# divortio/divortio-lz4

Measured on NVIDIA B200. Metric: lz4_block_roundtrip_throughput, higher is better.
Workload: dtype u8

## Files before the change

divortio-lz4_b200/csrc/api_launch.inc:

```
int compress_segmented(dlz4_ctx *ctx, const uint8_t *d_work, int64_t start, int64_t total, int64_t B, uint32_t n, bool linked,
                       const int32_t *init_table, uint8_t *d_comp, const uint64_t *d_coff, uint32_t *d_clen, cudaStream_t st,
                       int32_t *final_table = nullptr, const uint32_t *landed = nullptr, int32_t land_origin = 0,
                       uint32_t land_shift = 0);

int launch_compress(dlz4_ctx *ctx, const uint8_t *src, const uint64_t *src_off, const uint32_t *src_len, uint32_t n,
                    uint32_t max_len, const uint8_t *prefix, uint32_t prefix_len, const int32_t *init_table, uint8_t *dst,
                    const uint64_t *dst_off, uint32_t *comp_len, cudaStream_t st, uint32_t *counter = nullptr, bool dense = false) {
    if (n == 0) return DLZ4_OK;
    if (!counter) counter = ctx->d_counter;
    CK(cudaMemsetAsync(counter, 0, sizeof(uint32_t), st));
    if (init_table == nullptr) { prefix = nullptr; prefix_len = 0; }
    if (max_len <= 65536 && prefix_len == 0 && init_table == nullptr && ctx->split && n <= kMaxSplitBlocks) {
        const size_t region = (size_t)(counter - ctx->d_counter) % kGtabRegions;
        const uint64_t rstride = (uint64_t)max_len / 4 + 2;
        const size_t region_bytes = (((size_t)n * rstride * 8) * 9 / 8 + 255) & ~(size_t)255;
        if (ctx->rec.cap < region_bytes * kGtabRegions + 256) {
            CK(cudaDeviceSynchronize());
            CKS(reserve(ctx, ctx->rec, std::max(region_bytes, (size_t)ctx->rec.cap / kGtabRegions) * kGtabRegions));
        }
        const size_t per_region = ((ctx->rec.cap - 256) / kGtabRegions) & ~(size_t)255;
        uint64_t *recs = (uint64_t *)((uint8_t *)ctx->rec.p + region * per_region);
        uint32_t *nrec = ctx->d_nrec + region * (size_t)kMaxSplitBlocks;
        if (ctx->probe) CK(cudaEventRecord(ctx->evq[0], st));
        if (ctx->pw) {
            const int grid = (int)std::min<uint64_t>(n, (uint64_t)ctx->sm_count);
            const uint32_t lead = (uint32_t)ctx->pw_lead, ns = (uint32_t)ctx->pw_sleep;
            k_parse_pw<<<grid, kPwThreads, kPwSmemBytes, st>>>(src, src_off, src_len, n, recs, rstride, nrec, counter, lead, ns);
        } else
        {
            const int grid = (int)std::min<uint64_t>((n + kWarpsFresh16 - 1) / kWarpsFresh16, (uint64_t)ctx->sm_count);
            k_parse_fresh16<kWarpsFresh16><<<grid, kWarpsFresh16 * 32, kWarpsFresh16 * kHashEntries * 2, st>>>(
                src, src_off, src_len, n, recs, rstride, nrec, counter);
        }
        if (ctx->probe) CK(cudaEventRecord(ctx->evq[1], st));
        CK(cudaMemsetAsync(counter, 0, sizeof(uint32_t), st));
        const int egrid = (int)std::min<uint64_t>((n + kWarpsDecode - 1) / kWarpsDecode, (uint64_t)ctx->sm_count * 8);
        k_encode_blocks<kWarpsDecode><<<egrid, kWarpsDecode * 32, 0, st>>>(src, src_off, src_len, n, recs, rstride, nrec, dst, dst_off,
                                                                            comp_len, counter);
        if (ctx->probe) CK(cudaEventRecord(ctx->evq[2], st));
        ctx->launches++;
    } else if (max_len <= 65536 && prefix_len == 0 && init_table == nullptr && ctx->hybrid) {
        const size_t region = (size_t)(counter - ctx->d_counter) % kGtabRegions;
        const int grid = (int)std::min<uint64_t>(dense ? (n + kHyWarps - 1) / kHyWarps : n, (uint64_t)ctx->hy_grid);
        uint32_t active = dense ? (uint32_t)kHyWarps : (uint32_t)std::min<uint64_t>((n + grid - 1) / grid, (uint64_t)kHyWarps);
        if (ctx->hy_active) active = std::min<uint32_t>(active, (uint32_t)ctx->hy_active);
        k_compress_fresh16h<<<grid, kHyWarps * 32, kHySmemBytes, st>>>(
            src, src_off, src_len, n, dst, dst_off, comp_len, counter,
            ctx->d_gtabs + region * (size_t)ctx->hy_grid * kHyGlWarps * kHashEntries, active);
    } else if (max_len <= 4096 && prefix_len > 0 && init_table != nullptr && ctx->hybrid && prefix_len < 0x7FFF0000u) {
        const size_t region = (size_t)(counter - ctx->d_counter) % kGtabRegions;
        const int grid = (int)std::min<uint64_t>(dense ? (n + kHyWarps - 1) / kHyWarps : n, (uint64_t)ctx->hy_grid);
        const uint32_t active = dense ? (uint32_t)kHyWarps : (uint32_t)std::min<uint64_t>((n + grid - 1) / grid, (uint64_t)kHyWarps);
        k_compress_overlay<<<grid, kHyWarps * 32, kHySmemBytes, st>>>(
            src, src_off, src_len, n, prefix, prefix_len, init_table, dst, dst_off, comp_len, counter,
            ctx->d_gtabs + region * (size_t)ctx->hy_grid * kHyGlWarps * kHashEntries, active);
    } else {
        if (max_len > 65536 && prefix_len == 0 && init_table == nullptr && n <= 65536) {
            std::vector<uint64_t> off(n);
            std::vector<uint32_t> len(n);
            CK(cudaMemcpyAsync(off.data(), src_off, (size_t)n * 8, cudaMemcpyDeviceToHost, st));
            CK(cudaMemcpyAsync(len.data(), src_len, (size_t)n * 4, cudaMemcpyDeviceToHost, st));
            CK(cudaStreamSynchronize(st));
            const uint64_t B = len[0];
            bool uniform = B > 65536 && (B & (B - 1)) == 0 && off[0] + (uint64_t)n * B < 0x7FFFFFF0ull;
            for (uint32_t i = 0; uniform && i < n; ++i)
                uniform = off[i] == off[0] + (uint64_t)i * B && (len[i] == B || (i + 1 == n && len[i] <= B && len[i] > 0));
            if (uniform) {
                const int64_t total = (int64_t)(n - 1) * (int64_t)B + len[n - 1];
                return compress_segmented(ctx, src, (int64_t)off[0], total, (int64_t)B, n, false, nullptr, dst, dst_off, comp_len, st);
            }
        }
        const int grid = (int)std::min<uint64_t>((n + kWarpsGeneric32 - 1) / kWarpsGeneric32, (uint64_t)ctx->sm_count);
        k_compress_generic32<kWarpsGeneric32><<<grid, kWarpsGeneric32 * 32, kWarpsGeneric32 * (kHashEntries * 4 + kRingBytes), st>>>(
            src, src_off, src_len, n, prefix, prefix_len, init_table, dst, dst_off, comp_len, counter);
    }
    ctx->launches++;
    CK(cudaGetLastError());
    return DLZ4_OK;
}

int launch_decompress(dlz4_ctx *ctx, const uint8_t *src, const uint64_t *src_off, const uint32_t *src_len, uint32_t n,
                      uint8_t *dst, const uint64_t *dst_off, const uint32_t *dst_cap, const uint8_t *dict, uint32_t dict_len,
                      int hist_frame, const uint8_t *stored, uint32_t *out_len, uint8_t *status, cudaStream_t st,
                      uint32_t *counter = nullptr) {
    if (n == 0) return DLZ4_OK;
    if (!counter) counter = ctx->d_counter;
    CK(cudaMemsetAsync(counter, 0, sizeof(uint32_t), st));
    const int grid = hist_frame ? 1 : (int)std::min<uint64_t>((n + kWarpsDecode - 1) / kWarpsDecode, (uint64_t)ctx->sm_count * 8);
    if (dict_len)
        k_decompress_blocks<kWarpsDecode, true><<<grid, hist_frame ? 32 : kWarpsDecode * 32, 0, st>>>(src, src_off, src_len, n, dst, dst_off, dst_cap,
                                                                                                      dict, dict_len, hist_frame, stored, out_len, status, counter);
    else
        k_decompress_blocks<kWarpsDecode, false><<<grid, hist_frame ? 32 : kWarpsDecode * 32, 0, st>>>(src, src_off, src_len, n, dst, dst_off, dst_cap,
                                                                                                       dict, dict_len, hist_frame, stored, out_len, status, counter);
    ctx->launches++;
    CK(cudaGetLastError());
    return DLZ4_OK;
}

int launch_xxh32_batch(dlz4_ctx *ctx, const uint8_t *base, const uint64_t *off, const uint32_t *len, uint32_t n, uint32_t seed,
                       uint32_t *out, uint8_t *append_base, cudaStream_t st) {
    if (n == 0) return DLZ4_OK;
    const uint64_t threads = (uint64_t)n * 4;
    k_xxh32_batch<<<(unsigned)((threads + 255) / 256), 256, 0, st>>>(base, off, len, n, seed, out, append_base);
    ctx->launches++;
    CK(cudaGetLastError());
    return DLZ4_OK;
}

int launch_xxh32_stream(dlz4_ctx *ctx, const uint8_t *data, uint64_t len, uint32_t seed, uint32_t *out, cudaStream_t st) {
    k_xxh32_stream<1><<<1, 32, 0, st>>>(data, len, seed, out, nullptr, nullptr);
    ctx->launches++;
    CK(cudaGetLastError());
    return DLZ4_OK;
}
```

divortio-lz4_b200/csrc/dlz4_parse.cuh:

```cuda
#pragma once

namespace dlz4 {

__device__ __forceinline__ uint2 rec_pack(uint32_t pos, uint32_t ml, uint32_t offset) { return make_uint2(pos | (offset << 16), ml); }

template <class Tab>
__device__ uint32_t parse_block64_warp(const uint8_t *__restrict__ base, const int32_t start, const int32_t len, Tab &T,
                                       uint64_t *__restrict__ rec) {
    const uint32_t lane = lane_id();
    const uint32_t lt = (1u << lane) - 1u;
    const int32_t sEnd = start + len;
    const int32_t mflimit = sEnd - 12;
    const int32_t matchLimit = sEnd - 5;
    int32_t sIndex = start;
    uint32_t smc = 67;
    uint32_t nrec = 0;
    const SrcFlat S{base};

    const uint32_t A0 = (uint32_t)(reinterpret_cast<uintptr_t>(base) & 127u);
    const int32_t wlo = start - (int32_t)((A0 + (uint32_t)start) & 3u);
    const int32_t whi = sEnd;
    uint32_t R0 = 0, R1 = 0, R2 = 0, R3 = 0;
    uint32_t Lc = 0;
    bool cold = true;
// ... 88 lines not shown
            uint32_t mlxa = mla, mlxb = mlb;
            uint32_t cur = 0;
            while (hl < 64u) {
                const uint32_t pk = __shfl_sync(FULL, pack, hl);
                const uint32_t fld = (pk >> ((hl >> 1) & 16u)) & 0xFFFFu;
                uint32_t mlh = fld & 63u;
                uint32_t nxt = fld >> 6;
                if (mlh == 32u && matchLimit - (w + (int32_t)hl) > 32) {
                    const int32_t s0 = w + (int32_t)hl;
                    const int32_t m0 = __shfl_sync(FULL, (hl & 32u) ? candb : canda, hl);
                    for (int32_t eb = 32;; eb += 128) {
                        const int32_t q = s0 + eb + 4 * (int32_t)lane;
                        int32_t nv = matchLimit - q;
                        nv = nv > 4 ? 4 : nv;
                        int32_t eq = 0;
                        if (nv > 0) {
                            const uint32_t x = S.ld32(q) ^ S.ld32(m0 + eb + 4 * (int32_t)lane);
                            eq = x ? ((__ffs(x) - 1) >> 3) : 4;
                            eq = eq < nv ? eq : nv;
                        }
                        const uint32_t stop = __ballot_sync(FULL, eq < 4);
                        if (stop) {
                            const int l = __ffs(stop) - 1;
                            mlh = (uint32_t)(eb + 4 * l + __shfl_sync(FULL, eq, l));
                            break;
                        }
                    }
                    nxt = first_hit_from(hl + mlh);
                    if (lane == (hl & 31u)) { if (hl & 32u) mlxb = mlh; else mlxa = mlh; }
                }
                if (lane == (hl & 31u)) myhead |= 1u + (hl >> 5);
                cur = hl + mlh;
                hl = nxt;
            }
            const uint32_t stop = any_head ? trunc : min(trunc, dl0);
            const uint32_t Ha = __ballot_sync(FULL, myhead & 1u), Hb = __ballot_sync(FULL, myhead & 2u);
            const uint32_t enda = min(lane + mlxa, 255u), endb = min(lane + 32u + mlxb, 255u);
            const uint32_t ends = enda | (endb << 8);
            const uint32_t ma_lo = Ha & lt, mb_lo = Hb & lt;
            const int pha = ma_lo ? 31 - __clz(ma_lo) : -1;
            const int phb = mb_lo ? 63 - __clz(mb_lo) : (Ha ? 31 - __clz(Ha) : -1);
            const uint32_t ea = __shfl_sync(FULL, ends, pha & 31), eb2 = __shfl_sync(FULL, ends, phb & 31);
            const uint32_t end_pha = pha < 0 ? 0u : (ea & 255u);
            const uint32_t end_phb = phb < 0 ? 0u : (phb >= 32 ? eb2 >> 8 : eb2 & 255u);
            const bool ina = lane < end_pha, inb = lane + 32u < end_phb;
            const bool pra = lane < stop && !ina;
            const bool prb = lane + 32u < stop && !inb;
            if (conf) {
                if (lane < trunc) tab_set_raw(T, ha, pra ? taga : olda);
                if (lane + 32u < trunc) tab_set_raw(T, hb, prb ? tagb : oldb);
            } else {
                if (!pra) tab_set_raw(T, ha, olda);
                if (!prb) tab_set_raw(T, hb, oldb);
            }
            uint2 *const rec2 = reinterpret_cast<uint2 *>(rec) + nrec;
            const uint32_t prel = (uint32_t)(w - start) + lane;
            if (myhead & 1u) rec2[__popc(ma_lo)] = make_uint2(prel | (offa << 16), mlxa);
            if (myhead & 2u) rec2[__popc(Ha) + __popc(mb_lo)] = make_uint2((prel + 32u) | (offb << 16), mlxb);
            nrec += __popc(Ha) + __popc(Hb);
            if (cur < stop) {
                smc = (any_head ? 67u : smc) + (stop - cur);
                sIndex = w + (int32_t)stop;
            } else {
                smc = 67u;
                sIndex = w + (int32_t)cur;
            }
            __syncwarp();
            continue;
        }

        const uint32_t base_sum = skip_sum(smc);
        const int32_t p = sIndex + (int32_t)(skip_sum(smc + lane) - base_sum);
        const bool valid = p < mflimit;
        uint32_t seq = 0, h = 0x10000u + lane;
        int32_t cand = -1;
        if (valid) {
            seq = S.ld32(p);
            h = (seq * 2654435761u) >> 18;
            cand = T.get(h);
        }
        const uint32_t same = __match_any_sync(FULL, h);
        const uint32_t prev = same & lt;
        const int j = prev ? 31 - __clz(prev) : (int)lane;
        const int32_t pj = __shfl_sync(FULL, p, j);
        const uint32_t sj = __shfl_sync(FULL, seq, j);
        uint32_t cseq = sj;
        if (prev) cand = pj;
        const bool ok = valid && cand >= 0 && cand != p && (((uint32_t)(p - cand)) >> 16) == 0;
        if (ok && !prev) cseq = S.ld32(cand);
        const bool hit = ok && cseq == seq;
        const uint32_t hits = __ballot_sync(FULL, hit);
        const uint32_t vmask = __ballot_sync(FULL, valid);
        const int hl = __ffs(hits) - 1;
        const uint32_t commit = hits ? ((2u << hl) - 1u) : vmask;
        if (((commit >> lane) & 1u) && ((same & commit) >> lane) == 1u) T.put(h, p);
        __syncwarp();
        if (!hits) {
            if (vmask != FULL) break;
            sIndex += (int32_t)(skip_sum(smc + 32u) - base_sum);
            smc += 32u;
            continue;
        }
        const int32_t s0 = __shfl_sync(FULL, p, hl);
        const int32_t m0 = __shfl_sync(FULL, cand, hl);
        smc = 67;
        int32_t ml;
        for (int32_t eb = 4;; eb += 128) {
            const int32_t q = s0 + eb + 4 * (int32_t)lane;
            int32_t nv = matchLimit - q;
            nv = nv > 4 ? 4 : nv;
            int32_t eq = 0;
            if (nv > 0) {
                const uint32_t x = S.ld32(q) ^ S.ld32(m0 + eb + 4 * (int32_t)lane);
                eq = x ? ((__ffs(x) - 1) >> 3) : 4;
                eq = eq < nv ? eq : nv;
            }
            const uint32_t stop = __ballot_sync(FULL, eq < 4);
            if (stop) {
                const int l = __ffs(stop) - 1;
                ml = eb + 4 * l + __shfl_sync(FULL, eq, l);
                break;
            }
        }
        if (lane == 0) reinterpret_cast<uint2 *>(rec)[nrec] = rec_pack((uint32_t)(s0 - start), (uint32_t)ml, (uint32_t)(s0 - m0));
        ++nrec;
        sIndex = s0 + ml;
    }
    return nrec;
}

template <int WARPS>
__global__ void __launch_bounds__(WARPS * 32, 1)
k_parse_fresh16(const uint8_t *__restrict__ src, const uint64_t *__restrict__ src_off, const uint32_t *__restrict__ src_len,
                uint32_t nblocks, uint64_t *__restrict__ rec_base, uint64_t rec_stride ,
                uint32_t *__restrict__ nrec_out, uint32_t *counter) {
    extern __shared__ __align__(16) uint8_t smem[];
    const uint32_t lane = lane_id(), warp = threadIdx.x >> 5;
    uint16_t *tab = reinterpret_cast<uint16_t *>(smem) + warp * kHashEntries;
    for (;;) {
        const uint32_t b = next_block(counter, lane);
        if (b >= nblocks) break;
        const uint32_t len = src_len[b];
        if (len > 65536u) { if (lane == 0) nrec_out[b] = 0xFFFFFFFFu; continue; }
        uint4 *t4 = reinterpret_cast<uint4 *>(tab);
        for (uint32_t i = lane; i < kHashEntries * 2 / 16; i += 32) t4[i] = make_uint4(0, 0, 0, 0);
        __syncwarp();
        Tab16 T{tab, 0};
        const uint32_t n = parse_block64_warp(src + src_off[b], 0, (int32_t)len, T, rec_base + (uint64_t)b * rec_stride);
        if (lane == 0) nrec_out[b] = n;
        __syncwarp();
    }
}

template <int WARPS>
__global__ void __launch_bounds__(WARPS * 32)
k_encode_blocks(const uint8_t *__restrict__ src, const uint64_t *__restrict__ src_off, const uint32_t *__restrict__ src_len,
                uint32_t nblocks, const uint64_t *__restrict__ rec_base, uint64_t rec_stride, const uint32_t *__restrict__ nrec_in,
                uint8_t *__restrict__ dst, const uint64_t *__restrict__ dst_off, uint32_t *__restrict__ comp_len, uint32_t *counter) {
    const uint32_t lane = lane_id();
    const bool twice = nblocks <= 0x7FFFFFFFu;
    const uint32_t qlen = twice ? 2u * nblocks : nblocks;
    for (;;) {
        const uint32_t qi = next_block(counter, lane);
        if (qi >= qlen) break;
        const uint32_t b = qi < nblocks ? qi : qi - nblocks;
        const uint32_t n = nrec_in[b];
        if (twice && (n != 0xFFFFFFFFu && n >= 256u) != (qi < nblocks)) continue;
        if (n == 0xFFFFFFFFu) { if (lane == 0) comp_len[b] = 0xFFFFFFFFu; continue; }
        const uint8_t *in = src + src_off[b];
        const uint32_t len = src_len[b];
        const uint64_t *rec = rec_base + (uint64_t)b * rec_stride;
        uint8_t *out = dst + dst_off[b];
        uint32_t D = 0, prev_end = 0;
        for (uint32_t r0 = 0; r0 < n; r0 += 32) {
            const uint32_t i = r0 + lane;
            const bool have = i < n;
            const uint2 rc = have ? reinterpret_cast<const uint2 *>(rec)[i] : make_uint2(0u, 0u);
            const uint32_t pos = rc.x & 0xFFFFu, ml = rc.y, offset = rc.x >> 16;
            const uint32_t end = pos + ml;
            uint32_t pe = __shfl_up_sync(FULL, end, 1);
            if (lane == 0) pe = prev_end;
            const uint32_t lit = have ? pos - pe : 0u;
            const uint32_t code = ml - 4u;
            const uint32_t litx = lit >= 15u ? 1u + (lit - 15u) / 255u : 0u;
            const uint32_t mlx = have && code >= 15u ? 1u + (code - 15u) / 255u : 0u;
            const uint32_t size = have ? 3u + litx + lit + mlx : 0u;
            uint32_t incl = size;
#pragma unroll
            for (int o = 1; o < 32; o <<= 1) { const uint32_t y = __shfl_up_sync(FULL, incl, o); if (lane >= (uint32_t)o) incl += y; }
            uint32_t d = D + incl - size;
            if (have) {
                out[d++] = (uint8_t)(((lit < 15u ? lit : 15u) << 4) | (code < 15u ? code : 15u));
                if (lit >= 15u) {
                    uint32_t rest = lit - 15u;
                    while (rest >= 255u) { out[d++] = 255; rest -= 255u; }
                    out[d++] = (uint8_t)rest;
                }
            }
            const uint32_t lits_at = d;
            const bool longrun = have && lit > 24u;
            if (have && !longrun) {
                const uint8_t *s = in + pe;
                for (uint32_t k = 0; k < lit; ++k) out[d + k] = s[k];
            }
            for (uint32_t m = __ballot_sync(FULL, longrun); m; m &= m - 1u) {
                const int l = __ffs(m) - 1;
                const uint32_t o_ = __shfl_sync(FULL, lits_at, l), p_ = __shfl_sync(FULL, pe, l), n_ = __shfl_sync(FULL, lit, l);
                warp_copy(out + o_, in + p_, n_, lane);
            }
            if (have) {
                d += lit;
                out[d] = (uint8_t)offset;
                out[d + 1] = (uint8_t)(offset >> 8);
                d += 2;
                if (code >= 15u) {
                    uint32_t rest = code - 15u;
                    while (rest >= 255u) { out[d++] = 255; rest -= 255u; }
                    out[d] = (uint8_t)rest;
                }
            }
            D += __shfl_sync(FULL, incl, 31);
            const uint32_t last = min(n - r0, 32u) - 1u;
            prev_end = __shfl_sync(FULL, end, last);
        }
        __syncwarp();
        uint8_t *e = emit_literals(out + D, SrcFlat{in}, (int32_t)prev_end, len - prev_end, 0u, lane);
        if (lane == 0) comp_len[b] = (uint32_t)(e - out);
        __syncwarp();
    }
}

}
```

divortio-lz4_b200/csrc/dlz4_pw.cuh:

```cuda
#pragma once

namespace dlz4 {

constexpr int kPwChains = 7;
constexpr int kPwProducers = 2;
constexpr int kPwThreads = 8 * (1 + kPwProducers) * 32;
constexpr int kPwWin = 14;
constexpr uint32_t kPwTmemCols = 128;
constexpr int kPwCtl = 64;
constexpr int kPwChainBytes = kHashEntries * 2 + kPwCtl;
constexpr int kPwSmemBytes = kPwChains * kPwChainBytes + 16;
constexpr uint32_t kPwRingSmc = 160u;
constexpr uint32_t kPwDone = 0x80000000u, kPwSparse = 0x40000000u;
constexpr bool kPwPrefetch = true;
#ifndef DLZ4_PW_CAP
#define DLZ4_PW_CAP 32
#endif
constexpr uint32_t kPwCap = DLZ4_PW_CAP;

struct PwCtl {
    uint32_t w_pos;
    volatile uint32_t block;
    uint32_t ready[kPwWin];
};
static_assert(sizeof(PwCtl) <= kPwCtl, "PwCtl");

__device__ __forceinline__ void pw_bar(uint32_t id, uint32_t nthreads) {
    asm volatile("bar.sync %0, %1;" ::"r"(id), "r"(nthreads) : "memory");
}
__device__ __forceinline__ uint32_t pw_ld_acquire(const uint32_t *p) {
    uint32_t v;
    asm volatile("ld.acquire.cta.shared.u32 %0, [%1];" : "=r"(v) : "r"((uint32_t)__cvta_generic_to_shared(p)) : "memory");
    return v;
}
__device__ __forceinline__ void pw_st_release(uint32_t *p, const uint32_t v) {
    asm volatile("st.release.cta.shared.u32 [%0], %1;" ::"r"((uint32_t)__cvta_generic_to_shared(p)), "r"(v) : "memory");
}
__device__ __forceinline__ void pw_st_release2(uint32_t *p, const uint32_t v0, const uint32_t v1) {
    asm volatile("st.release.cta.shared.v2.u32 [%0], {%1, %2};" ::"r"((uint32_t)__cvta_generic_to_shared(p)), "r"(v0), "r"(v1) : "memory");
}
__device__ __forceinline__ void pw_prefetch(const void *p) { asm volatile("prefetch.global.L1 [%0];" ::"l"(p)); }
__device__ __forceinline__ void tm_fence_before() { asm volatile("tcgen05.fence::before_thread_sync;" ::: "memory"); }
__device__ __forceinline__ void tm_fence_after() { asm volatile("tcgen05.fence::after_thread_sync;" ::: "memory"); }
__device__ __forceinline__ void tm_st8(const uint32_t t, const uint32_t x0, const uint32_t y0, const uint32_t z0, const uint32_t x1,
                                       const uint32_t y1, const uint32_t z1) {
    asm volatile("tcgen05.st.sync.aligned.32x32b.x8.b32 [%0], {%1, %2, %3, %3, %4, %5, %6, %6};\n\t"
                 "tcgen05.wait::st.sync.aligned;" ::"r"(t), "r"(x0), "r"(y0), "r"(z0), "r"(x1), "r"(y1), "r"(z1) : "memory");
}
__device__ __forceinline__ void tm_ld4(const uint32_t t, uint32_t &x, uint32_t &y, uint32_t &z) {
    uint32_t u;
    asm volatile("tcgen05.ld.sync.aligned.32x32b.x4.b32 {%0, %1, %2, %3}, [%4];\n\t"
                 "tcgen05.wait::ld.sync.aligned;\n\t"
                 "tcgen05.fence::before_thread_sync;" : "=r"(x), "=r"(y), "=r"(z), "=r"(u) : "r"(t) : "memory");
}
__device__ __forceinline__ void tm_ld2(const uint32_t t, uint32_t &x, uint32_t &y) {
    asm volatile("tcgen05.ld.sync.aligned.32x32b.x2.b32 {%0, %1}, [%2];\n\t"
                 "tcgen05.wait::ld.sync.aligned;\n\t"
                 "tcgen05.fence::before_thread_sync;" : "=r"(x), "=r"(y) : "r"(t) : "memory");
}
__device__ __forceinline__ uint32_t pw_ws(const uint32_t w) { return w - (uint32_t)kPwWin * ((w * 74899u) >> 20); }
__device__ __forceinline__ void pw_wait_ready(const PwCtl *ctl, const uint32_t ws, const uint32_t w, const uint32_t ns) {
    while (!__all_sync(FULL, pw_ld_acquire(ctl->ready + ws) == w + 1u)) __nanosleep(ns);
    tm_fence_after();
}
__device__ __forceinline__ uint32_t pw_resolve(const uint32_t ml, const uint32_t lane, uint32_t &exitp) {
    uint32_t n = ml == kPwCap ? 255u : lane + (ml ? ml : 1u);
    uint32_t m = 1u << lane;
#pragma unroll
    for (int r = 0; r < 5; ++r) {
        const uint32_t mj = __shfl_sync(FULL, m, n), nj = __shfl_sync(FULL, n, n);
        if (n < 32u) { m |= mj; n = nj; }
    }
    exitp = n;
    return m;
}

__device__ __forceinline__ uint32_t pw_extend(const uint8_t *__restrict__ base, int32_t s0, int32_t m0, int32_t eb,
                                              int32_t matchLimit, uint32_t lane) {
    const int32_t back = s0 - m0;
    auto round4 = [&](int32_t e0, uint32_t &res) -> bool {
        const int32_t q = s0 + e0 + 4 * (int32_t)lane;
        int32_t nv = matchLimit - q;
        nv = nv > 4 ? 4 : nv;
        int32_t eq = 0;
        if (nv > 0) {
            const uint32_t x = ld32u(base + q) ^ ld32u(base + q - back);
            const int32_t e = x ? ((__ffs(x) - 1) >> 3) : 4;
            eq = e < nv ? e : nv;
        }
        const uint32_t stop = __ballot_sync(FULL, eq < 4);
        if (!stop) return false;
        const int l = __ffs(stop) - 1;
        res = (uint32_t)(e0 + 4 * l + __shfl_sync(FULL, eq, l));
        return true;
    };
    uint32_t res = 0;
    if (round4(eb, res)) return res;
    eb += 128;
    const uint32_t mis = (uint32_t)(reinterpret_cast<uintptr_t>(base + s0 + eb) & 15u);
    if (mis) {
        if (round4(eb, res)) return res;
        eb += 128 - (int32_t)mis;
        eb -= 112;
    }
    const uint8_t *cb = base + s0 + eb - back;
    const uint32_t cmis = (uint32_t)(reinterpret_cast<uintptr_t>(cb) & 15u);
    const uint32_t wsel = cmis >> 2, bsh = (cmis & 3u) * 8u;
    for (;; eb += 2048) {
        uint32_t eqb[4];
#pragma unroll
        for (int u = 0; u < 4; ++u) {
            const int32_t q = s0 + eb + 512 * u + 16 * (int32_t)lane;
            int32_t nv = matchLimit - q;
            nv = nv > 16 ? 16 : nv;
            eqb[u] = 0;
            if (nv > 0) {
                const uint4 a = __ldg(reinterpret_cast<const uint4 *>(base + q));
                const uint4 *cp = reinterpret_cast<const uint4 *>(base + q - back - (int32_t)cmis);
                const uint4 c0 = __ldg(cp), c1 = __ldg(cp + 1);
                uint32_t v[8] = {c0.x, c0.y, c0.z, c0.w, c1.x, c1.y, c1.z, c1.w};
                uint32_t t[5];
#pragma unroll
                for (int i = 0; i < 5; ++i) t[i] = wsel == 0 ? v[i] : wsel == 1 ? v[i + 1] : wsel == 2 ? v[i + 2] : v[i + 3];
                const uint32_t x0 = a.x ^ __funnelshift_r(t[0], t[1], bsh), x1 = a.y ^ __funnelshift_r(t[1], t[2], bsh);
                const uint32_t x2 = a.z ^ __funnelshift_r(t[2], t[3], bsh), x3 = a.w ^ __funnelshift_r(t[3], t[4], bsh);
                uint32_t e = x0 ? ((uint32_t)(__ffs(x0) - 1) >> 3) : x1 ? 4u + ((uint32_t)(__ffs(x1) - 1) >> 3)
                           : x2 ? 8u + ((uint32_t)(__ffs(x2) - 1) >> 3) : x3 ? 12u + ((uint32_t)(__ffs(x3) - 1) >> 3) : 16u;
                eqb[u] = e < (uint32_t)nv ? e : (uint32_t)nv;
            }
        }
#pragma unroll
        for (int u = 0; u < 4; ++u) {
            const uint32_t stop = __ballot_sync(FULL, eqb[u] < 16u);
            if (stop) { const int l = __ffs(stop) - 1; return (uint32_t)(eb + 512 * u + 16 * l) + __shfl_sync(FULL, eqb[u], l); }
        }
    }
}


__device__ __forceinline__ uint32_t pw_count32(const uint4 &q0, const uint4 &q1, const uint4 &q2, const uint32_t cs, const uint32_t *Sw) {
    uint32_t v[12] = {q0.x, q0.y, q0.z, q0.w, q1.x, q1.y, q1.z, q1.w, q2.x, q2.y, q2.z, q2.w};
    const bool s8 = (cs & 8u) != 0, s4 = (cs & 4u) != 0;
#pragma unroll
    for (int k = 0; k < 10; ++k) v[k] = s8 ? v[k + 2] : v[k];
#pragma unroll
    for (int k = 0; k < 9; ++k) v[k] = s4 ? v[k + 1] : v[k];
    const uint32_t csh = (cs & 3u) * 8u;
    uint32_t x[8];
#pragma unroll
    for (int k = 0; k < 8; ++k) x[k] = Sw[k] ^ __funnelshift_r(v[k], v[k + 1], csh);
    const bool h4 = (x[0] | x[1] | x[2] | x[3]) == 0u;
    const uint32_t y0 = h4 ? x[4] : x[0], y1 = h4 ? x[5] : x[1], y2 = h4 ? x[6] : x[2], y3 = h4 ? x[7] : x[3];
    const bool h2 = (y0 | y1) == 0u;
    const uint32_t z0 = h2 ? y2 : y0, z1 = h2 ? y3 : y1;
    const bool h1 = z0 == 0u;
    const uint32_t zz = h1 ? z1 : z0;
    return (h4 ? 16u : 0u) + (h2 ? 8u : 0u) + (h1 ? 4u : 0u) + (zz ? ((uint32_t)(__ffs(zz) - 1) >> 3) : 4u);
}

__device__ __forceinline__ void pw_produce2(const uint8_t *__restrict__ base, const uint32_t k, const bool two, const uint16_t *tab,
                                            const uint32_t tcol, PwCtl *ctl, const uint32_t lane) {
    const uint32_t pa = 32u * k + lane, pb = pa + 32u;
    const uintptr_t ba = reinterpret_cast<uintptr_t>(base);
    const uint32_t a = (uint32_t)(ba & 3u) + pa;
    const uint32_t *wp = reinterpret_cast<const uint32_t *>(ba & ~(uintptr_t)3) + (a >> 2);
    const uint32_t sh = (a & 3u) * 8u;
    uint32_t w[17];
#pragma unroll
    for (int i = 0; i < 9; ++i) w[i] = __ldg(wp + i);
#pragma unroll
    for (int i = 9; i < 17; ++i) w[i] = two ? __ldg(wp + i) : 0u;
    uint32_t S[16];
#pragma unroll
    for (int i = 0; i < 16; ++i) S[i] = __funnelshift_r(w[i], w[i + 1], sh);
    const uint32_t ha = (S[0] * 2654435761u) >> 18, hb = (S[8] * 2654435761u) >> 18;
    const uint32_t seena = *reinterpret_cast<const volatile uint16_t *>(tab + ha);
    const uint32_t seenb = *reinterpret_cast<const volatile uint16_t *>(tab + hb);
    const bool oka = seena != pa, okb = two && seenb != pb;
// ... 146 lines not shown
            sIndex = (int32_t)(wbase + (uint32_t)__ffs(PM & ~below) - 1u);
            const uint32_t hx = __shfl_sync(FULL, h, (uint32_t)sIndex - wbase);
            const uint32_t cand = tab[hx];
            __syncwarp();
            if (lane == 0) tab[hx] = (uint16_t)sIndex;
            __syncwarp();
            uint32_t mlx = 0;
            if (cand != (uint32_t)sIndex) mlx = pw_extend(base, sIndex, (int32_t)cand, 0, matchLimit, lane);
            if (mlx >= 4u) {
                if (lane == 0) rec2[nrec] = rec_pack((uint32_t)sIndex, mlx, (uint32_t)sIndex - cand);
                ++nrec;
                sIndex += (int32_t)mlx;
                smc = 67u;
            } else {
                sIndex += (int32_t)(smc >> 6);
                ++smc;
            }
            PT_MARK(4) PT_COUNT(10, 1)
            continue;
        }
        if (smc <= kPwRingSmc && sIndex < rlimit) {
            const uint32_t bs = skip_sum(smc);
            const int32_t p = sIndex + (int32_t)(skip_sum(smc + lane) - bs);
            const bool valid = p < rlimit;
            if (pub != (uint32_t)sIndex) { pub = (uint32_t)sIndex; if (lane == 0) pw_st_release(&ctl->w_pos, pub); }
            const uint32_t w0 = (uint32_t)sIndex >> 5;
            const uint32_t wl = (uint32_t)min(__shfl_sync(FULL, p, 31), rlimit - 1) >> 5;
            uint32_t lo = 0, ye = 0;
            for (uint32_t w = w0; w <= wl; ++w) {
                const uint32_t ws = pw_ws(w);
                pw_wait_ready(ctl, ws, w, 20);
                uint32_t xw, yw;
                tm_ld2(tcol + 4u * ws, xw, yw);
                xw = __shfl_sync(FULL, xw, (uint32_t)p & 31u);
                yw = __shfl_sync(FULL, yw, (uint32_t)p & 31u);
                if (((uint32_t)p >> 5) == w) { lo = xw; ye = yw; }
            }
            const uint32_t seen = ye & 0xFFFFu;
            const uint32_t h = lo & 0x3FFFu, ml = (lo >> 14) & 127u;
            const uint32_t cur = tab[h];
            const uint32_t claim = __ballot_sync(FULL, valid && ml != 0u);
            const uint32_t f = claim ? (uint32_t)__ffs(claim) - 1u : 32u;
            const bool active = valid && lane <= f;
            const uint32_t tag = (uint32_t)p & 0xFFFFu;
            __syncwarp();
            if (active) tab[h] = (uint16_t)tag;
            __syncwarp();
            const uint32_t r = active ? (uint32_t)tab[h] : tag;
            const uint32_t bad = __ballot_sync(FULL, active && (r != tag || cur != seen));
            if (!bad) {
                if (claim) {
                    const int32_t pf = sIndex + (int32_t)(skip_sum(smc + f) - bs);
                    const uint32_t curf = __shfl_sync(FULL, cur, f);
                    uint32_t mlf = __shfl_sync(FULL, ml, f);
                    if (mlf == kPwCap) mlf = pw_extend(base, pf, (int32_t)curf, (int32_t)kPwCap, matchLimit, lane);
                    if (lane == 0) rec2[nrec] = rec_pack((uint32_t)pf, mlf, (uint32_t)pf - curf);
                    ++nrec;
                    sIndex = pf + (int32_t)mlf;
                    smc = 67u;
                } else {
                    const uint32_t nv = (uint32_t)__popc(__ballot_sync(FULL, valid));
                    sIndex += (int32_t)(skip_sum(smc + nv) - bs);
                    smc += nv;
                }
                PT_MARK(2) PT_COUNT(11, 1)
                continue;
            }
            const uint32_t inv = (active && r != tag) ? min((uint32_t)p, r) : 0xFFFFFFFFu;
            const uint32_t cutpos = __reduce_min_sync(FULL, inv);
            const uint32_t grp = __ballot_sync(FULL, active && (uint32_t)p <= cutpos);
            const uint32_t stale = __ballot_sync(FULL, active && cur != seen);
            const uint32_t c = min((uint32_t)__popc(grp), stale ? (uint32_t)__ffs(stale) - 1u : 32u);
            if (active && lane >= c) tab[h] = (uint16_t)cur;
            __syncwarp();
            if (active && lane < c) tab[h] = (uint16_t)tag;
            __syncwarp();
            if (c != 0u) {
                sIndex += (int32_t)(skip_sum(smc + c) - bs);
                smc += c;
                PT_MARK(2) PT_COUNT(11, 1)
                continue;
            }
            const uint32_t h0 = __shfl_sync(FULL, h, 0);
            const uint32_t cand = tab[h0];
            __syncwarp();
            if (lane == 0) tab[h0] = (uint16_t)sIndex;
            __syncwarp();
            uint32_t ml0 = 0;
            if (cand != (uint32_t)sIndex) ml0 = pw_extend(base, sIndex, (int32_t)cand, 0, matchLimit, lane);
            if (ml0 >= 4u) {
                if (lane == 0) rec2[nrec] = rec_pack((uint32_t)sIndex, ml0, (uint32_t)sIndex - cand);
                ++nrec;
                sIndex += (int32_t)ml0;
                smc = 67u;
            } else {
                sIndex += (int32_t)(smc >> 6);
                ++smc;
            }
            PT_MARK(2) PT_COUNT(11, 1)
            continue;
        }

        if (smc > kPwRingSmc && sIndex < rlimit) {
            const uint32_t v = (uint32_t)sIndex | kPwSparse;
            if (pub != v) { pub = v; if (lane == 0) pw_st_release(&ctl->w_pos, pub); }
        }
        const uint32_t base_sum = skip_sum(smc);
        const int32_t p = sIndex + (int32_t)(skip_sum(smc + lane) - base_sum);
        const bool valid = p < mflimit;
        uint32_t seq = 0, h = 0x10000u + lane;
        int32_t cand = -1;
        if (valid) {
            seq = S.ld32(p);
            h = (seq * 2654435761u) >> 18;
            cand = T.get(h);
        }
        const uint32_t same = __match_any_sync(FULL, h);
        const uint32_t prev = same & lt;
        const int j = prev ? 31 - __clz(prev) : (int)lane;
        const int32_t pj = __shfl_sync(FULL, p, j);
        const uint32_t sj = __shfl_sync(FULL, seq, j);
        uint32_t cseq = sj;
        if (prev) cand = pj;
        const bool ok = valid && cand >= 0 && cand != p && (((uint32_t)(p - cand)) >> 16) == 0;
        if (ok && !prev) cseq = S.ld32(cand);
        const bool hit = ok && cseq == seq;
        const uint32_t hits = __ballot_sync(FULL, hit);
        const uint32_t vmask = __ballot_sync(FULL, valid);
        const int hl = __ffs(hits) - 1;
        const uint32_t commit = hits ? ((2u << hl) - 1u) : vmask;
        if (((commit >> lane) & 1u) && ((same & commit) >> lane) == 1u) T.put(h, p);
        __syncwarp();
        if (!hits) {
            if (vmask != FULL) break;
            sIndex += (int32_t)(skip_sum(smc + 32u) - base_sum);
            smc += 32u;
            PT_MARK(3) PT_COUNT(12, 1)
            continue;
        }
        const int32_t s0 = __shfl_sync(FULL, p, hl);
        const int32_t m0 = __shfl_sync(FULL, cand, hl);
        smc = 67;
        const uint32_t ml = pw_extend(base, s0, m0, 4, matchLimit, lane);
        if (lane == 0) rec2[nrec] = rec_pack((uint32_t)s0, ml, (uint32_t)(s0 - m0));
        ++nrec;
        sIndex = s0 + (int32_t)ml;
        PT_MARK(3) PT_COUNT(12, 1)
    }
    PT_MARK(5)
    PT_FLUSH
    return nrec;
}

__global__ void __launch_bounds__(kPwThreads, 1)
k_parse_pw(const uint8_t *__restrict__ src, const uint64_t *__restrict__ src_off, const uint32_t *__restrict__ src_len,
           uint32_t nblocks, uint64_t *__restrict__ rec_base, uint64_t rec_stride ,
           uint32_t *__restrict__ nrec_out, uint32_t *counter, uint32_t lead,
           uint32_t full_ns ) {
    extern __shared__ __align__(16) uint8_t smem[];
    constexpr uint32_t kRoles = 1 + kPwProducers;
    constexpr uint32_t kTeam = kRoles * 32;
    const uint32_t lane = lane_id(), warp = threadIdx.x >> 5;
    const uint32_t quarter = warp & 3u, tslot = (warp >> 2) / kRoles, role = (warp >> 2) % kRoles;
    const uint32_t chain = quarter + 4u * tslot;
    uint32_t *const taddr_smem = reinterpret_cast<uint32_t *>(smem + kPwChains * kPwChainBytes);
    if (warp == 0) {
        asm volatile("tcgen05.alloc.cta_group::1.sync.aligned.shared::cta.b32 [%0], %1;\n\t"
                     "tcgen05.relinquish_alloc_permit.cta_group::1.sync.aligned;"
                     ::"r"((uint32_t)__cvta_generic_to_shared(taddr_smem)), "r"(kPwTmemCols) : "memory");
    }
    tm_fence_before();
    __syncthreads();
    tm_fence_after();
    const uint32_t taddr = *taddr_smem;
    const uint32_t tcol = taddr + ((32u * quarter) << 16) + tslot * (uint32_t)(kPwWin * 4);
    if (chain < (uint32_t)kPwChains) {
        const uint32_t tid = role * 32u + lane;
        uint8_t *const cb = smem + (size_t)chain * kPwChainBytes;
        uint16_t *const tab = reinterpret_cast<uint16_t *>(cb);
        PwCtl *const ctl = reinterpret_cast<PwCtl *>(cb + kHashEntries * 2);
        const uint32_t bar = 1u + chain;
        uint32_t first = chain * gridDim.x + blockIdx.x;
        const uint32_t qbase = gridDim.x * (uint32_t)kPwChains;
        bool have_first = true;
        for (;;) {
            pw_bar(bar, kTeam);
            if (role == 0 && lane == 0) {
                uint32_t b;
                if (have_first) b = first; else b = qbase + atomicAdd(counter, 1u);
                ctl->block = b < nblocks ? b : 0xFFFFFFFFu;
                ctl->w_pos = 0u;
            }
            have_first = false;
            pw_bar(bar, kTeam);
            const uint32_t b = ctl->block;
            if (b == 0xFFFFFFFFu) break;
            const uint32_t len = src_len[b];
            if (len > 65536u) {
                if (role == 0 && lane == 0) nrec_out[b] = 0xFFFFFFFFu;
                continue;
            }
            {
                uint4 *z = reinterpret_cast<uint4 *>(cb);
                for (uint32_t i = tid; i < kHashEntries * 2 / 16; i += kTeam) z[i] = make_uint4(0, 0, 0, 0);
                if (tid < (uint32_t)kPwWin) ctl->ready[tid] = 0u;
            }
            pw_bar(bar, kTeam);
            const uint8_t *base = src + src_off[b];
            uint64_t *const rec = rec_base + (uint64_t)b * rec_stride;
            const uint32_t nwin = len >= 112u ? (len - 111u) / 32u + 1u : 0u;
            if (role == 0) {
                const uint32_t n = pw_walker(base, (int32_t)len, nwin, tab, tcol, ctl, rec, lane);
                if (lane == 0) {
                    nrec_out[b] = n;
                    pw_st_release(&ctl->w_pos, kPwDone);
                }
            } else {
                pw_producer(base, nwin, lead, role - 1u, tab, tcol, ctl, lane, full_ns);
            }
        }
    }
    tm_fence_before();
    __syncthreads();
    tm_fence_after();
    if (warp == 0)
        asm volatile("tcgen05.dealloc.cta_group::1.sync.aligned.b32 %0, %1;" ::"r"(taddr), "r"(kPwTmemCols) : "memory");
}

}
```

Measured before the change: 78.47.

## Fuse LZ4 sequence encoding into the pipelined parse kernel via shared work pool

Removes the separate k_encode_blocks launch when the pipelined-walker parse path is enabled. Parsed blocks are instead published to a shared-memory pool and encoded by four extra encoder warps per CTA, with the walker encoding a block itself when the pool is full. The encode code is factored into a shared warp-level helper. The aim is to drop a kernel launch plus the counter memset and to overlap encoding with parsing. In exchange the parse CTA gets more threads, spin-polling, and more complex termination logic.

```diff
diff --git a/divortio-lz4_b200/csrc/api_launch.inc b/divortio-lz4_b200/csrc/api_launch.inc
--- a/divortio-lz4_b200/csrc/api_launch.inc
+++ b/divortio-lz4_b200/csrc/api_launch.inc
@@ -25,20 +25,21 @@
         if (ctx->pw) {
             const int grid = (int)std::min<uint64_t>(n, (uint64_t)ctx->sm_count);
             const uint32_t lead = (uint32_t)ctx->pw_lead, ns = (uint32_t)ctx->pw_sleep;
-            k_parse_pw<<<grid, kPwThreads, kPwSmemBytes, st>>>(src, src_off, src_len, n, recs, rstride, nrec, counter, lead, ns);
-        } else
-        {
+            k_parse_pw<<<grid, kPwThreads, kPwSmemBytes, st>>>(src, src_off, src_len, n, recs, rstride, nrec, dst, dst_off, comp_len,
+                                                               counter, lead, ns);
+            if (ctx->probe) { CK(cudaEventRecord(ctx->evq[1], st)); CK(cudaEventRecord(ctx->evq[2], st)); }
+        } else {
             const int grid = (int)std::min<uint64_t>((n + kWarpsFresh16 - 1) / kWarpsFresh16, (uint64_t)ctx->sm_count);
             k_parse_fresh16<kWarpsFresh16><<<grid, kWarpsFresh16 * 32, kWarpsFresh16 * kHashEntries * 2, st>>>(
                 src, src_off, src_len, n, recs, rstride, nrec, counter);
+            if (ctx->probe) CK(cudaEventRecord(ctx->evq[1], st));
+            CK(cudaMemsetAsync(counter, 0, sizeof(uint32_t), st));
+            const int egrid = (int)std::min<uint64_t>((n + kWarpsDecode - 1) / kWarpsDecode, (uint64_t)ctx->sm_count * 8);
+            k_encode_blocks<kWarpsDecode><<<egrid, kWarpsDecode * 32, 0, st>>>(src, src_off, src_len, n, recs, rstride, nrec, dst, dst_off,
+                                                                                comp_len, counter);
+            if (ctx->probe) CK(cudaEventRecord(ctx->evq[2], st));
+            ctx->launches++;
         }
-        if (ctx->probe) CK(cudaEventRecord(ctx->evq[1], st));
-        CK(cudaMemsetAsync(counter, 0, sizeof(uint32_t), st));
-        const int egrid = (int)std::min<uint64_t>((n + kWarpsDecode - 1) / kWarpsDecode, (uint64_t)ctx->sm_count * 8);
-        k_encode_blocks<kWarpsDecode><<<egrid, kWarpsDecode * 32, 0, st>>>(src, src_off, src_len, n, recs, rstride, nrec, dst, dst_off,
-                                                                            comp_len, counter);
-        if (ctx->probe) CK(cudaEventRecord(ctx->evq[2], st));
-        ctx->launches++;
     } else if (max_len <= 65536 && prefix_len == 0 && init_table == nullptr && ctx->hybrid) {
         const size_t region = (size_t)(counter - ctx->d_counter) % kGtabRegions;
         const int grid = (int)std::min<uint64_t>(dense ? (n + kHyWarps - 1) / kHyWarps : n, (uint64_t)ctx->hy_grid);
diff --git a/divortio-lz4_b200/csrc/dlz4_parse.cuh b/divortio-lz4_b200/csrc/dlz4_parse.cuh
--- a/divortio-lz4_b200/csrc/dlz4_parse.cuh
+++ b/divortio-lz4_b200/csrc/dlz4_parse.cuh
@@ -264,6 +264,65 @@
     }
 }
 
+__device__ __forceinline__ uint32_t encode_block_warp(const uint8_t *__restrict__ in, const uint32_t len, const uint2 *rec,
+                                                      const uint32_t n, uint8_t *__restrict__ out, const uint32_t lane) {
+    uint32_t D = 0, prev_end = 0;
+    for (uint32_t r0 = 0; r0 < n; r0 += 32) {
+        const uint32_t i = r0 + lane;
+        const bool have = i < n;
+        const uint2 rc = have ? rec[i] : make_uint2(0u, 0u);
+        const uint32_t pos = rc.x & 0xFFFFu, ml = rc.y, offset = rc.x >> 16;
+        const uint32_t end = pos + ml;
+        uint32_t pe = __shfl_up_sync(FULL, end, 1);
+        if (lane == 0) pe = prev_end;
+        const uint32_t lit = have ? pos - pe : 0u;
+        const uint32_t code = ml - 4u;
+        const uint32_t litx = lit >= 15u ? 1u + (lit - 15u) / 255u : 0u;
+        const uint32_t mlx = have && code >= 15u ? 1u + (code - 15u) / 255u : 0u;
+        const uint32_t size = have ? 3u + litx + lit + mlx : 0u;
+        uint32_t incl = size;
+#pragma unroll
+        for (int o = 1; o < 32; o <<= 1) { const uint32_t y = __shfl_up_sync(FULL, incl, o); if (lane >= (uint32_t)o) incl += y; }
+        uint32_t d = D + incl - size;
+        if (have) {
+            out[d++] = (uint8_t)(((lit < 15u ? lit : 15u) << 4) | (code < 15u ? code : 15u));
+            if (lit >= 15u) {
+                uint32_t rest = lit - 15u;
+                while (rest >= 255u) { out[d++] = 255; rest -= 255u; }
+                out[d++] = (uint8_t)rest;
+            }
+        }
+        const uint32_t lits_at = d;
+        const bool longrun = have && lit > 24u;
+        if (have && !longrun) {
+            const uint8_t *s = in + pe;
+            for (uint32_t k = 0; k < lit; ++k) out[d + k] = s[k];
+        }
+        for (uint32_t m = __ballot_sync(FULL, longrun); m; m &= m - 1u) {
+            const int l = __ffs(m) - 1;
+            const uint32_t o_ = __shfl_sync(FULL, lits_at, l), p_ = __shfl_sync(FULL, pe, l), n_ = __shfl_sync(FULL, lit, l);
+            warp_copy(out + o_, in + p_, n_, lane);
+        }
+        if (have) {
+            d += lit;
+            out[d] = (uint8_t)offset;
+            out[d + 1] = (uint8_t)(offset >> 8);
+            d += 2;
+            if (code >= 15u) {
+                uint32_t rest = code - 15u;
+                while (rest >= 255u) { out[d++] = 255; rest -= 255u; }
+                out[d] = (uint8_t)rest;
+            }
+        }
+        D += __shfl_sync(FULL, incl, 31);
+        const uint32_t last = min(n - r0, 32u) - 1u;
+        prev_end = __shfl_sync(FULL, end, last);
+    }
+    __syncwarp();
+    uint8_t *e = emit_literals(out + D, SrcFlat{in}, (int32_t)prev_end, len - prev_end, 0u, lane);
+    return (uint32_t)(e - out);
+}
+
 template <int WARPS>
 __global__ void __launch_bounds__(WARPS * 32)
 k_encode_blocks(const uint8_t *__restrict__ src, const uint64_t *__restrict__ src_off, const uint32_t *__restrict__ src_len,
@@ -279,65 +338,9 @@
         const uint32_t n = nrec_in[b];
         if (twice && (n != 0xFFFFFFFFu && n >= 256u) != (qi < nblocks)) continue;
         if (n == 0xFFFFFFFFu) { if (lane == 0) comp_len[b] = 0xFFFFFFFFu; continue; }
-        const uint8_t *in = src + src_off[b];
-        const uint32_t len = src_len[b];
-        const uint64_t *rec = rec_base + (uint64_t)b * rec_stride;
-        uint8_t *out = dst + dst_off[b];
-        uint32_t D = 0, prev_end = 0;
-        for (uint32_t r0 = 0; r0 < n; r0 += 32) {
-            const uint32_t i = r0 + lane;
-            const bool have = i < n;
-            const uint2 rc = have ? reinterpret_cast<const uint2 *>(rec)[i] : make_uint2(0u, 0u);
-            const uint32_t pos = rc.x & 0xFFFFu, ml = rc.y, offset = rc.x >> 16;
-            const uint32_t end = pos + ml;
-            uint32_t pe = __shfl_up_sync(FULL, end, 1);
-            if (lane == 0) pe = prev_end;
-            const uint32_t lit = have ? pos - pe : 0u;
-            const uint32_t code = ml - 4u;
-            const uint32_t litx = lit >= 15u ? 1u + (lit - 15u) / 255u : 0u;
-            const uint32_t mlx = have && code >= 15u ? 1u + (code - 15u) / 255u : 0u;
-            const uint32_t size = have ? 3u + litx + lit + mlx : 0u;
-            uint32_t incl = size;
-#pragma unroll
-            for (int o = 1; o < 32; o <<= 1) { const uint32_t y = __shfl_up_sync(FULL, incl, o); if (lane >= (uint32_t)o) incl += y; }
-            uint32_t d = D + incl - size;
-            if (have) {
-                out[d++] = (uint8_t)(((lit < 15u ? lit : 15u) << 4) | (code < 15u ? code : 15u));
-                if (lit >= 15u) {
-                    uint32_t rest = lit - 15u;
-                    while (rest >= 255u) { out[d++] = 255; rest -= 255u; }
-                    out[d++] = (uint8_t)rest;
-                }
-            }
-            const uint32_t lits_at = d;
-            const bool longrun = have && lit > 24u;
-            if (have && !longrun) {
-                const uint8_t *s = in + pe;
-                for (uint32_t k = 0; k < lit; ++k) out[d + k] = s[k];
-            }
-            for (uint32_t m = __ballot_sync(FULL, longrun); m; m &= m - 1u) {
-                const int l = __ffs(m) - 1;
-                const uint32_t o_ = __shfl_sync(FULL, lits_at, l), p_ = __shfl_sync(FULL, pe, l), n_ = __shfl_sync(FULL, lit, l);
-                warp_copy(out + o_, in + p_, n_, lane);
-            }
-            if (have) {
-                d += lit;
-                out[d] = (uint8_t)offset;
-                out[d + 1] = (uint8_t)(offset >> 8);
-                d += 2;
-                if (code >= 15u) {
-                    uint32_t rest = code - 15u;
-                    while (rest >= 255u) { out[d++] = 255; rest -= 255u; }
-                    out[d] = (uint8_t)rest;
-                }
-            }
-            D += __shfl_sync(FULL, incl, 31);
-            const uint32_t last = min(n - r0, 32u) - 1u;
-            prev_end = __shfl_sync(FULL, end, last);
-        }
-        __syncwarp();
-        uint8_t *e = emit_literals(out + D, SrcFlat{in}, (int32_t)prev_end, len - prev_end, 0u, lane);
-        if (lane == 0) comp_len[b] = (uint32_t)(e - out);
+        const uint32_t c = encode_block_warp(src + src_off[b], src_len[b], reinterpret_cast<const uint2 *>(rec_base + (uint64_t)b * rec_stride),
+                                             n, dst + dst_off[b], lane);
+        if (lane == 0) comp_len[b] = c;
         __syncwarp();
     }
 }
diff --git a/divortio-lz4_b200/csrc/dlz4_pw.cuh b/divortio-lz4_b200/csrc/dlz4_pw.cuh
--- a/divortio-lz4_b200/csrc/dlz4_pw.cuh
+++ b/divortio-lz4_b200/csrc/dlz4_pw.cuh
@@ -4,12 +4,14 @@
 
 constexpr int kPwChains = 7;
 constexpr int kPwProducers = 2;
-constexpr int kPwThreads = 8 * (1 + kPwProducers) * 32;
+constexpr int kPwXEnc = 4;
+constexpr int kPwThreads = (8 * (1 + kPwProducers) + kPwXEnc) * 32;
 constexpr int kPwWin = 14;
 constexpr uint32_t kPwTmemCols = 128;
 constexpr int kPwCtl = 64;
 constexpr int kPwChainBytes = kHashEntries * 2 + kPwCtl;
-constexpr int kPwSmemBytes = kPwChains * kPwChainBytes + 16;
+constexpr int kPwPool = 64;
+constexpr int kPwSmemBytes = kPwChains * kPwChainBytes + 16 + kPwPool * 4;
 constexpr uint32_t kPwRingSmc = 160u;
 constexpr uint32_t kPwDone = 0x80000000u, kPwSparse = 0x40000000u;
 constexpr bool kPwPrefetch = true;
@@ -24,6 +26,7 @@
     uint32_t ready[kPwWin];
 };
 static_assert(sizeof(PwCtl) <= kPwCtl, "PwCtl");
+static_assert(kPwPool == 64, "pw_publish / pw_claim: two pool words per lane");
 
 __device__ __forceinline__ void pw_bar(uint32_t id, uint32_t nthreads) {
     asm volatile("bar.sync %0, %1;" ::"r"(id), "r"(nthreads) : "memory");
@@ -476,10 +479,46 @@
     return nrec;
 }
 
+__device__ __forceinline__ bool pw_publish(uint32_t *pool, const uint32_t b, const uint32_t lane) {
+    __syncwarp();
+    for (;;) {
+        const volatile uint32_t *vp = pool;
+        const uint32_t f0 = __ballot_sync(FULL, vp[lane] == 0u), f1 = __ballot_sync(FULL, vp[lane + 32u] == 0u);
+        if (!(f0 | f1)) return false;
+        const uint32_t i = f0 ? (uint32_t)__ffs(f0) - 1u : 31u + (uint32_t)__ffs(f1);
+        uint32_t ok = 0;
+        if (lane == 0) { __threadfence_block(); ok = atomicCAS(pool + i, 0u, b + 1u) == 0u; }
+        if (__shfl_sync(FULL, ok, 0)) return true;
+    }
+}
+__device__ __forceinline__ uint32_t pw_claim(uint32_t *pool, const uint32_t lane) {
+    for (;;) {
+        const volatile uint32_t *vp = pool;
+        const uint32_t t0 = __ballot_sync(FULL, vp[lane] != 0u), t1 = __ballot_sync(FULL, vp[lane + 32u] != 0u);
+        if (!(t0 | t1)) return 0u;
+        const uint32_t i = t0 ? (uint32_t)__ffs(t0) - 1u : 31u + (uint32_t)__ffs(t1);
+        uint32_t v = 0;
+        if (lane == 0) { v = atomicExch(pool + i, 0u); __threadfence_block(); }
+        v = __shfl_sync(FULL, v, 0);
+        __syncwarp();
+        if (v) return v;
+    }
+}
+__device__ __forceinline__ void pw_encode(const uint8_t *__restrict__ src, const uint64_t *__restrict__ src_off,
+                                          const uint32_t *__restrict__ src_len, const uint64_t *rec_base, const uint64_t rec_stride,
+                                          const uint32_t *nrec, uint8_t *__restrict__ dst, const uint64_t *__restrict__ dst_off,
+                                          uint32_t *__restrict__ comp_len, const uint32_t b, const uint32_t lane) {
+    const uint32_t c = encode_block_warp(src + src_off[b], src_len[b], reinterpret_cast<const uint2 *>(rec_base + (uint64_t)b * rec_stride),
+                                         nrec[b], dst + dst_off[b], lane);
+    if (lane == 0) comp_len[b] = c;
+    __syncwarp();
+}
+
 __global__ void __launch_bounds__(kPwThreads, 1)
 k_parse_pw(const uint8_t *__restrict__ src, const uint64_t *__restrict__ src_off, const uint32_t *__restrict__ src_len,
            uint32_t nblocks, uint64_t *__restrict__ rec_base, uint64_t rec_stride ,
-           uint32_t *__restrict__ nrec_out, uint32_t *counter, uint32_t lead,
+           uint32_t *__restrict__ nrec_out, uint8_t *__restrict__ dst, const uint64_t *__restrict__ dst_off,
+           uint32_t *__restrict__ comp_len, uint32_t *counter, uint32_t lead,
            uint32_t full_ns ) {
     extern __shared__ __align__(16) uint8_t smem[];
     constexpr uint32_t kRoles = 1 + kPwProducers;
@@ -488,11 +527,15 @@
     const uint32_t quarter = warp & 3u, tslot = (warp >> 2) / kRoles, role = (warp >> 2) % kRoles;
     const uint32_t chain = quarter + 4u * tslot;
     uint32_t *const taddr_smem = reinterpret_cast<uint32_t *>(smem + kPwChains * kPwChainBytes);
+    uint32_t *const teams_done = taddr_smem + 1;
+    uint32_t *const pool = taddr_smem + 4;
     if (warp == 0) {
         asm volatile("tcgen05.alloc.cta_group::1.sync.aligned.shared::cta.b32 [%0], %1;\n\t"
                      "tcgen05.relinquish_alloc_permit.cta_group::1.sync.aligned;"
                      ::"r"((uint32_t)__cvta_generic_to_shared(taddr_smem)), "r"(kPwTmemCols) : "memory");
     }
+    if (threadIdx.x < (uint32_t)kPwPool) pool[threadIdx.x] = 0u;
+    if (threadIdx.x == (uint32_t)kPwPool) *teams_done = 0u;
     tm_fence_before();
     __syncthreads();
     tm_fence_after();
@@ -521,7 +564,7 @@
             if (b == 0xFFFFFFFFu) break;
             const uint32_t len = src_len[b];
             if (len > 65536u) {
-                if (role == 0 && lane == 0) nrec_out[b] = 0xFFFFFFFFu;
+                if (role == 0 && lane == 0) comp_len[b] = 0xFFFFFFFFu;
                 continue;
             }
             {
@@ -539,10 +582,25 @@
                     nrec_out[b] = n;
                     pw_st_release(&ctl->w_pos, kPwDone);
                 }
+                if (!pw_publish(pool, b, lane)) pw_encode(src, src_off, src_len, rec_base, rec_stride, nrec_out, dst, dst_off, comp_len, b, lane);
             } else {
                 pw_producer(base, nwin, lead, role - 1u, tab, tcol, ctl, lane, full_ns);
             }
         }
+        if (role == 0 && lane == 0) { __threadfence_block(); atomicAdd(teams_done, 1u); }
+    }
+    for (;;) {
+        uint32_t v = pw_claim(pool, lane);
+        if (v == 0u) {
+            const bool fin = pw_ld_acquire(teams_done) == (uint32_t)kPwChains;
+            v = pw_claim(pool, lane);
+            if (v == 0u) {
+                if (fin) break;
+                __nanosleep(512);
+                continue;
+            }
+        }
+        pw_encode(src, src_off, src_len, rec_base, rec_stride, nrec_out, dst, dst_off, comp_len, v - 1u, lane);
     }
     tm_fence_before();
     __syncthreads();
```

New measurement: 79.46, median of 6. 1.3% higher.
